# danping/CoSLAM

Hardware: AMD Instinct MI355X
Metric: frames/sec for track+local-BA loop, 8 cams 640x480 x 2000 feats (one frame = all 8 cameras) (higher is better)
Workload: dtype f32 (KLT, f16 pyramid storage) + f64 (pose, BA)

## Files before the change

coslam_amd/csrc/poseupdate.hip:

```cpp
#include <atomic>
#include <cstdlib>
#include <vector>

#include "cs_common.h"
#include "project_dev.h"
#include "triangulate_dev.h"
#include "history_view.h"
#include "register_rows_dev.h"
#include "small_ops.h"

#pragma clang fp contract(off)

namespace {

constexpr int PU_MAX_CAMS = 16;
constexpr int PU_MAX_HIST = 512;
constexpr int PU_MAX_STORE = 1 << 16;
constexpr int PU_LPS = 8;

struct PuArgs {
    int nCams, N, nMap, cam0, nCamsRun;
    int gateBlocks, dynBlocksPerCam;
    const int* pointFeat;
    const double* R;
// ... 2745 lines not shown
        return CS_ERR_INVALID;
    }
    if (!q.M || !q.cov || !q.pointFeat || !q.slot || !q.m || !q.var || !q.dist || !q.flags || q.M != d_mapPts || q.cov != d_mapCov ||
        q.pointFeat != d_pointFeat) {
        cs_set_error("cs_register_revisit_rounds_dev: the pass needs every table, and its map, covariances and feature table are the ones refined");
        return CS_ERR_INVALID;
    }
    if (nMap < 1 || cap < 1 || cap > RV_MAX_ROWS || nRounds < 1 || nRounds > 8 || kinds < 1 || kinds > 3 || mapBase < 0 || !(tolPix >= 0) ||
        !d_mapPts || !d_mapCov || !d_mergeCache || !d_mergeable || !d_rvLists || !d_rvCounts || !d_visitLoop || !d_nextLoop || !d_mapFlags ||
        !d_pointFeat || !d_slot2map || !d_attached || !d_regOut || !d_decideScratch || !d_curList || !d_curCount || !d_featRef ||
        (long long)nCams * N > RD_FEAT || (long long)nCams * nMap * nCams > 0x7fffffffLL) {
        cs_set_error("cs_register_revisit_rounds_dev: bad arguments (1..%d rows, 1..8 rounds, kinds 1..3, every table)", RV_MAX_ROWS);
        return CS_ERR_INVALID;
    }
    if (h->count < 1 || curFrame != h->lastFrame) {
        cs_set_error("cs_register_revisit_rounds_dev: the history's newest entry must be frame %d (it holds %d frame(s), the newest %d)", curFrame,
                     h->count, h->lastFrame);
        return CS_ERR_INVALID;
    }
    RrArgs A;
    memset((void*)&A, 0, sizeof(A));
    for (int c = 0; c < nCams; ++c) {
        const cs_register_cam& rc = regCams[c];
        if (!rc.K || !rc.R || !rc.t || !rc.xy || !rc.state || !rc.slot2map) {
            cs_set_error("cs_register_revisit_rounds_dev: null pointer in search camera %d", c);
            return CS_ERR_INVALID;
        }
        if (!cams[c].K || !cams[c].iK || !cams[c].trackSpan) {
            cs_set_error("cs_register_revisit_rounds_dev: null pointer in camera %d (K, iK, trackSpan are read)", c);
            return CS_ERR_INVALID;
        }
        if (!d_slot2map[c]) {
            cs_set_error("cs_register_revisit_rounds_dev: null slot2map of camera %d", c);
            return CS_ERR_INVALID;
        }
        A.rcam[c] = rc;
    }
    A.nRounds = nRounds, A.W = W, A.H = H, A.lists = d_rvLists, A.rvCounts = d_rvCounts;
    A.pass = q;
    A.pass.P = cap, A.pass.list = nullptr;
    MgCore& G = A.mg.a;
    G.cam0 = 0, G.nCams = nCams, G.N = N, G.P = nMap, G.H = h->H, G.head = h->head, G.nHist = hist_walk(h);
    G.sigma = pixelErrVar, G.M = d_mapPts, G.cov = d_mapCov, G.slot = q.slot, G.out = d_mergeable;
    G.histXY = h->xy, G.histR = h->R, G.histT = h->t;
    A.mg.W = hist_walk(h), A.mg.count = h->count, A.mg.curFrame = h->lastFrame, A.mg.epoch = h->tailEpoch, A.mg.fromMin = h->tailFromMin;
    A.mg.tolPix = tolPix, A.mg.cache = (MgCache*)d_mergeCache, A.mg.counts = nullptr, A.mg.flags = q.flags;
    RvArgs& V = A.rv;
    V.nCams = nCams, V.N = N, V.P = nMap, V.cap = cap, V.mapBase = mapBase, V.kinds = kinds, V.nextLoop = d_nextLoop, V.visitLoop = d_visitLoop;
    V.slot = q.slot, V.flags = q.flags, V.mergeable = d_mergeable, V.mapFlags = d_mapFlags, V.pointFeat = d_pointFeat;
    for (int c = 0; c < nCams; ++c) V.slot2map[c] = d_slot2map[c];
    V.attached = d_attached, V.regOut = d_regOut, V.curList = d_curList, V.curCount = d_curCount, V.curCap = curCap, V.counts = d_rvCnt;
    V.nextLoopW = d_nextLoop, V.overflow = d_rvCounts + nRounds;
    V.debug = cs_debug_get(CS_DBG_MERGE_PRINT) == 1;
    int* scr = (int*)d_decideScratch + (size_t)nCams * nMap + nMap;
    for (int k = 0; k < 3; ++k) V.owner[k] = scr, scr += (size_t)nCams * N;
    ArArgs& R = A.ar;
    R.nMap = nMap, R.featRef = (const int4*)d_featRef, R.mapPts = d_mapPts, R.mapCov = d_mapCov, R.sigma = pixelErrVar;
    R.refine = 1, R.select = d_regOut, R.selectW = d_regOut, R.clearSelect = 1;
    R.segPool = h->segPool, R.segCap = h->segCap, R.curFrame = h->lastFrame, R.stored = h->count < h->H ? h->count : h->H;
    R.nCams = nCams, R.N = N, R.H = h->H, R.head = h->head, R.nHist = hist_walk(h);
    R.histXY = h->xy, R.histR = h->R, R.histT = h->t, R.cen = h->cen;
    R.F.nCams = nCams, R.F.N = N, R.F.nMap = nMap, R.F.curFrame = curFrame, R.F.segCap = h->segCap;
    R.F.pointFeat = d_pointFeat, R.F.featRef = (int4*)d_featRef, R.F.refStatic = d_refStatic, R.F.segPool = h->segPool, R.F.segCount = h->segCount;
    R.F.counts = d_frefCounts;
    for (int c = 0; c < nCams; ++c) R.cam[c] = cams[c];
    CS_HIP(hipSetDevice(h->device));
    hipStream_t s = (hipStream_t)hip_stream;
    const int MC = nCams <= 8 ? 8 : RD_MAX_CAMS;
    const size_t lds = sizeof(double) * 12 * (size_t)A.mg.W + (cap > RR_THREADS ? sizeof(int) * (size_t)(MC + 1) * RV_MAX_ROWS : 0);
    size_t ldsMax = 0;
    if (const int rc = MC == 8 ? rr_dynamic_lds_limit<8>(h->device, &ldsMax) : rr_dynamic_lds_limit<RD_MAX_CAMS>(h->device, &ldsMax)) return rc;
    if (lds > ldsMax) {
        cs_set_error("cs_register_revisit_rounds_dev: %zu B of LDS (a history window of %d frames, lists of %d rows, %d cameras) where the "
                     "launch may carry %zu", lds, A.mg.W, cap, nCams, ldsMax);
        return CS_ERR_INVALID;
    }
    if (nMap > h->aliveCap) {
        if (h->alive) CS_HIP(hipFree(h->alive));
        h->alive = nullptr, h->aliveCap = 0;
        CS_HIP(hipMalloc((void**)&h->alive, (size_t)nMap));
        CS_HIP(hipMemsetAsync(h->alive, 1, (size_t)nMap, s));
        h->aliveCap = nMap;
    }
    R.F.alive = h->alive;
    hist_centres(h, s);
    if (MC == 8)
        hipLaunchKernelGGL(k_revisit_rounds<8>, dim3(1), dim3(RR_THREADS), lds, s, A);
    else
        hipLaunchKernelGGL(k_revisit_rounds<RD_MAX_CAMS>, dim3(1), dim3(RR_THREADS), lds, s, A);
    CS_HIP(hipGetLastError());
    return CS_OK;
}

extern "C" int cs_track_history_segments(const cs_track_history* h, cs_feat_seg** d_pool, int* cap, int** d_count) {
    if (!h) {
        cs_set_error("cs_track_history_segments: null handle");
        return CS_ERR_INVALID;
    }
    if (d_pool) *d_pool = (cs_feat_seg*)h->segPool;
    if (cap) *cap = h->segCap;
    if (d_count) *d_count = h->segCount;
    return CS_OK;
}

extern "C" int cs_track_history_segment_counts(const cs_track_history* h, int* counts) {
    if (!h || !counts) {
        cs_set_error("cs_track_history_segment_counts: bad arguments");
// ... 332 lines not shown
```

coslam_amd/csrc/register.hip:

```cpp
#include "cs_common.h"
#include "register_rows_dev.h"

#include <cfloat>

#pragma clang fp contract(off)

namespace {


struct RgArgs {
    int nCams, N, W, H, nPass, cam0;
    cs_register_pass pass[2];
    cs_register_cam cam[RG_MAX_CAMS];
};


constexpr int RG_WAVES = 8;
constexpr int RG_ROWS = RG_WAVES > 6 ? RG_WAVES : 6;
constexpr int RG_CHUNK = 512;

__global__ __launch_bounds__(64 * RG_WAVES) void k_register_search(RgArgs A) {
    extern __shared__ double lds[];
    CS_POSE_STREAM_PRIO();
    const int lane = threadIdx.x & 63, wave = threadIdx.x >> 6;
// ... 242 lines not shown
        const cs_register_cam& q = cams[c];
        if (!q.K || !q.R || !q.t || !q.xy || !q.state || !q.slot2map) {
            cs_set_error("cs_register_search_passes_dev: null pointer in camera %d", c);
            return CS_ERR_INVALID;
        }
        A.cam[c] = q;
    }
    CS_HIP(hipSetDevice(device));
    const int CH = N < RG_CHUNK ? N : RG_CHUNK;
    const size_t ldsBytes = (size_t)2 * CH * sizeof(double) + (size_t)RG_ROWS * 64 * sizeof(double) + (size_t)RG_WAVES * 64 * sizeof(int);
    hipLaunchKernelGGL(k_register_search, dim3((unsigned)((maxP + 63) / 64), (unsigned)nCamsRun, (unsigned)nPass), dim3(64 * RG_WAVES), ldsBytes,
                       (hipStream_t)hip_stream, A);
    CS_CHECK_LAUNCH();
    return CS_OK;
}

extern "C" int cs_register_search_dev(int device, void* hip_stream, int nCams, const cs_register_cam* cams, int N, int W, int H,
                                      int P, const double* d_M, const double* d_cov, const int* d_pointFeat, double sigmaSearch,
                                      double maxDist, double sigmaMerge, int* d_slot, double* d_m, double* d_var, double* d_dist,
                                      int* d_flags) {
    int rc = check_args("cs_register_search_dev", nCams, cams, N, W, H, P, sigmaSearch, maxDist, sigmaMerge);
    if (rc != CS_OK) return rc;
    if (P == 0) return CS_OK;
    if (!d_M || !d_cov || !d_pointFeat || !d_slot || !d_m || !d_var || !d_dist || !d_flags) {
        cs_set_error("cs_register_search_dev: null pointer");
        return CS_ERR_INVALID;
    }
    cs_register_pass q;
    memset(&q, 0, sizeof(q));
    q.P = P, q.sigmaSearch = sigmaSearch, q.maxDist = maxDist, q.sigmaMerge = sigmaMerge;
    q.M = d_M, q.cov = d_cov, q.pointFeat = d_pointFeat, q.slot = d_slot, q.m = d_m, q.var = d_var, q.dist = d_dist, q.flags = d_flags;
    return cs_register_search_passes_dev(device, hip_stream, nCams, cams, N, W, H, 1, &q);
}

namespace {

struct RdArgs {
    int nCams, N, P, mapBase, nSweeps, onlyCam, kinds;
    const int* slot;
    const int* flags;
    const unsigned char* mergeable;
    const unsigned char* mapFlags;
    int* pointFeat;
    int* slot2map[RD_MAX_CAMS];
    unsigned char* attached;
    unsigned char* regged;
    int* code;
    int* base;
    int* owner[3];
    int* counts;
    int* unconverged;
    int* timeouts;
    int* callFlag;
    int* changed;
    int* bar;
    int* rvLists;
    int* rvCounts;
    int rvCap, nRounds;
    int* visitLoop;
    int* nextLoop;
};
constexpr int RD_MAX_SWEEPS = 64;

__global__ __launch_bounds__(256) void k_decide_prepare(RdArgs A) {
    const int k = blockIdx.x * 256 + threadIdx.x, C = A.nCams, nFeat = C * A.N;
    for (int f = k; f < nFeat; f += gridDim.x * 256) A.owner[0][f] = RD_INF, A.owner[1][f] = RD_INF, A.owner[2][f] = RD_INF;
    if (k < 4 && A.counts) A.counts[k] = k == 2 ? A.nSweeps : (k == 3 ? 1 : 0);
    if (k == 0) *A.callFlag = 0, *A.bar = 0;
    if (k < RD_MAX_SWEEPS) A.changed[k] = 0;
    if (A.rvLists) {
        for (int f = k; f < A.nRounds * A.rvCap; f += gridDim.x * 256) A.rvLists[f] = -1;
        if (k < A.nRounds) A.rvCounts[k] = 0;
    }
    if (k >= A.P * C) return;
    const int p = k / C, i = k - p * C;
    A.attached[k] = 0;
    if (i == 0) A.regged[p] = 0;
    int code = -1;
    const unsigned char fl = A.mapFlags[p] & (CS_MAP_DYNAMIC | CS_MAP_FALSE | CS_MAP_UNCERTAIN);
    const int kind = (fl == 0 && (A.kinds & 1)) ? 0 : ((fl == CS_MAP_DYNAMIC && (A.kinds & 2)) ? 1 : -1);
    if (A.pointFeat[k] < 0 && kind >= 0) {
        const int s = A.slot[k];
        if (s >= 0 && s < A.N && ((A.flags[k] >> 1) & 1) == kind) {
            code = i * A.N + s;
            if (A.slot2map[i][s] >= 0) code |= RD_INIT_MAPPED;
            if (A.mergeable[k] == 1) code |= RD_CAN_MERGE;
        }
    }
    A.code[(size_t)i * A.P + p] = code;
    if (i == 0) {
        int ofirst = -1;
        for (int q = C - 1; q >= 0; --q)
            if (A.pointFeat[(size_t)p * C + q] >= 0) ofirst = q;
        if (A.onlyCam >= 0) ofirst = A.pointFeat[(size_t)p * C + A.onlyCam] >= 0 ? 0 : -1;
        A.base[p] = (ofirst >= 0 && kind >= 0) ? (ofirst * A.P + p) * C : -1;
    }
}
__global__ __launch_bounds__(256) void k_decide_sweep(RdArgs A, const int* __restrict__ prev, int* __restrict__ next, int* __restrict__ clear,
                                                      const int* __restrict__ prev2, int mode) {
    const int p = blockIdx.x * 256 + threadIdx.x, C = A.nCams, nFeat = C * A.N;
    if (clear)
        for (int f = p; f < nFeat; f += gridDim.x * 256) clear[f] = RD_INF;
    if (mode == 1 && prev2) {
        int ch = 0;
        for (int f = p; f < nFeat; f += gridDim.x * 256) ch |= prev[f] != prev2[f];
        if (ch) {
            if (A.counts) A.counts[3] = 0;
            if (atomicExch(A.callFlag, 1) == 0) atomicAdd(A.unconverged, 1);
        }
    }
    if (p >= A.P) return;
    const int base = A.base[p];
    if (base < 0) return;
    int code[RD_MAX_CAMS], own[RD_MAX_CAMS];
#pragma unroll
    for (int i = 0; i < RD_MAX_CAMS; ++i) code[i] = i < C ? A.code[(size_t)i * A.P + p] : -1;
#pragma unroll
    for (int i = 0; i < RD_MAX_CAMS; ++i) own[i] = code[i] >= 0 ? prev[code[i] & RD_FEAT] : RD_INF;
    bool go = true, reg = false;
    int nAtt = 0;
#pragma unroll
    for (int i = 0; i < RD_MAX_CAMS; ++i) {
        if (go && code[i] >= 0) {
            const int ord = base + i, f = code[i] & RD_FEAT;
            if ((code[i] & RD_INIT_MAPPED) || own[i] < ord) {
                go = false;
            } else if (code[i] & RD_CAN_MERGE) {
                if (mode == 0) {
                    atomicMin(&next[f], ord);
                } else if (own[i] == ord) {
                    const int s = f - i * A.N;
                    A.slot2map[i][s] = A.mapBase + p;
                    A.pointFeat[(size_t)p * C + i] = s;
                    A.attached[(size_t)p * C + i] = 1;
                    reg = true, ++nAtt;
                }
            }
        }
    }
    if (mode == 1 && reg) {
        A.regged[p] = 1;
        if (A.counts) atomicAdd(A.counts, nAtt), atomicAdd(A.counts + 1, 1);
    }
}

__device__ __forceinline__ bool rd_grid_barrier(int* ctr, int target) {
    __syncthreads();
    __shared__ int ok;
    if (threadIdx.x == 0) {
        __threadfence();
        atomicAdd(ctr, 1);
        const long long t0 = wall_clock64();
        int good = 1;
        while (__hip_atomic_load(ctr, __ATOMIC_ACQUIRE, __HIP_MEMORY_SCOPE_AGENT) < target) {
            __builtin_amdgcn_s_sleep(2);
            if (wall_clock64() - t0 > 2000000LL) {
                good = 0;
                break;
            }
        }
        ok = good;
    }
    __syncthreads();
    return ok != 0;
}

__global__ __launch_bounds__(256) void k_decide_settle(RdArgs A) {
    const int p = blockIdx.x * 256 + threadIdx.x, C = A.nCams, nFeat = C * A.N, nB = gridDim.x, stride = nB * 256;
    const int base = p < A.P ? A.base[p] : -1;
    int code[RD_MAX_CAMS];
#pragma unroll
    for (int i = 0; i < RD_MAX_CAMS; ++i) code[i] = (base >= 0 && i < C) ? A.code[(size_t)i * A.P + p] : -1;
    int arrivals = 0, k = 0;
    bool settled = false, alive = true;
    const int* fin = A.owner[0];
    for (; k < RD_MAX_SWEEPS; ++k) {
        const int* prev = A.owner[k % 3];
        int* next = A.owner[(k + 1) % 3];
        int* clear = A.owner[(k + 2) % 3];
        for (int f = p; f < nFeat; f += stride) rd_st(clear + f, RD_INF);
        if (base >= 0) {
            bool go = true;
#pragma unroll
            for (int i = 0; i < RD_MAX_CAMS; ++i) {
                if (go && code[i] >= 0) {
                    const int ord = base + i, f = code[i] & RD_FEAT;
                    if ((code[i] & RD_INIT_MAPPED) || rd_ld(prev + f) < ord) {
                        go = false;
                    } else if (code[i] & RD_CAN_MERGE) {
                        atomicMin(&next[f], ord);
                    }
                }
            }
        }
        arrivals += nB;
        if (!rd_grid_barrier(A.bar, arrivals)) {
            alive = false;
            break;
        }
        int ch = 0;
        for (int f = p; f < nFeat; f += stride) ch |= rd_ld(next + f) != rd_ld(prev + f);
        if (__syncthreads_or(ch) && threadIdx.x == 0) atomicOr(A.changed + k, 1);
        arrivals += nB;
        if (!rd_grid_barrier(A.bar, arrivals)) {
            alive = false;
            break;
        }
        fin = next;
        if (rd_ld(A.changed + k) == 0) {
            settled = true;
            ++k;
            break;
        }
    }
    if (p == 0 && A.counts) A.counts[2] = k, A.counts[3] = settled ? 1 : 0;
    if (!settled && p == 0) atomicAdd(A.unconverged, 1);
    if (!alive && p == 0) atomicAdd(A.timeouts, 1);
    if (!alive || base < 0) return;
    bool go = true, reg = false;
    int nAtt = 0;
#pragma unroll
    for (int i = 0; i < RD_MAX_CAMS; ++i) {
        if (go && code[i] >= 0) {
            const int ord = base + i, f = code[i] & RD_FEAT, own = rd_ld(fin + f);
            if ((code[i] & RD_INIT_MAPPED) || own < ord) {
                go = false;
            } else if ((code[i] & RD_CAN_MERGE) && own == ord) {
                const int s2 = f - i * A.N;
                A.slot2map[i][s2] = A.mapBase + p;
                A.pointFeat[(size_t)p * C + i] = s2;
                A.attached[(size_t)p * C + i] = 1;
                reg = true, ++nAtt;
            }
        }
    }
    if (reg) {
        A.regged[p] = 1;
        if (A.counts) atomicAdd(A.counts, nAtt), atomicAdd(A.counts + 1, 1);
        if (A.rvLists && A.onlyCam < 0) {
            const int last = (base / C) / A.P;
            A.visitLoop[p] = last;
            int b = -1;
            for (int c = C - 1; c > last; --c)
                if (A.pointFeat[(size_t)p * C + c] >= 0) b = c;
            if (b >= 0) {
                const int q = atomicAdd(A.rvCounts, 1);
                if (q < A.rvCap) A.rvLists[q] = p, A.nextLoop[p] = b;
                else atomicAdd(A.rvCounts + A.nRounds, 1);
            }
        }
    }
}

struct RvListArgs {
    int nCams, P, cap, firstRound;
    const int* pointFeat;
    const unsigned char* attached;
    unsigned char* regIn;
    int keepIn;
    unsigned char* regOutClear;
    int* visitLoop;
    int* nextLoop;
    int* list;
    int* counts;
};
__global__ __launch_bounds__(1024) void k_revisit_list(RvListArgs A) {
    __shared__ int sCount;
    const int tid = threadIdx.x, C = A.nCams;
    if (tid == 0) sCount = 0;
    __syncthreads();
    for (int p = tid; p < A.P; p += 1024) {
        if (A.regOutClear) A.regOutClear[p] = 0;
        if (!A.regIn[p]) continue;
        if (!A.keepIn) A.regIn[p] = 0;
        int last;
        if (A.firstRound) {
            last = -1;
            for (int c = C - 1; c >= 0; --c)
                if (A.pointFeat[(size_t)p * C + c] >= 0 && !A.attached[(size_t)p * C + c]) last = c;
            A.visitLoop[p] = last;
        } else {
            last = A.visitLoop[p];
        }
        if (last < 0) continue;
        int b = -1;
        for (int c = C - 1; c > last; --c)
            if (A.pointFeat[(size_t)p * C + c] >= 0) b = c;
        if (b < 0) continue;
        const int k = atomicAdd(&sCount, 1);
        if (k < A.cap) A.list[k] = p, A.nextLoop[p] = b;
    }
    __syncthreads();
    const int n = sCount < A.cap ? sCount : A.cap;
    for (int k = n + tid; k < A.cap; k += 1024) A.list[k] = -1;
    if (tid == 0 && A.counts) {
        A.counts[0] = n;
        if (sCount > A.cap) atomicAdd(A.counts + 1, sCount - A.cap);
    }
}

template <int MC>
__global__ __launch_bounds__(1024) void k_revisit_decide(RvArgs A) {
    if (A.listCount && *A.listCount == 0) return;
// ... 3 lines not shown
}

extern "C" int cs_register_revisit_list_dev(int device, void* hip_stream, int nCams, int P, int cap, int firstRound, const int* d_pointFeat,
                                            const unsigned char* d_attached, unsigned char* d_regIn, int keepIn, unsigned char* d_regOutClear,
                                            int* d_visitLoop, int* d_nextLoop, int* d_list, int* d_counts) {
    if (nCams < 1 || nCams > RD_MAX_CAMS || P < 1 || cap < 1 || cap > RV_MAX_ROWS || !d_pointFeat || !d_attached || !d_regIn || d_regOutClear == d_regIn || !d_visitLoop || !d_nextLoop ||
        !d_list) {
        cs_set_error("cs_register_revisit_list_dev: bad arguments (1..%d cameras, 1..%d rows)", RD_MAX_CAMS, RV_MAX_ROWS);
        return CS_ERR_INVALID;
    }
    RvListArgs A;
    A.nCams = nCams, A.P = P, A.cap = cap, A.firstRound = firstRound ? 1 : 0, A.pointFeat = d_pointFeat, A.attached = d_attached;
    A.regIn = d_regIn, A.keepIn = keepIn ? 1 : 0, A.regOutClear = d_regOutClear, A.visitLoop = d_visitLoop, A.nextLoop = d_nextLoop, A.list = d_list, A.counts = d_counts;
    CS_HIP(hipSetDevice(device));
    hipLaunchKernelGGL(k_revisit_list, dim3(1), dim3(1024), 0, (hipStream_t)hip_stream, A);
    CS_CHECK_LAUNCH();
    return CS_OK;
}

extern "C" int cs_register_revisit_decide_dev(int device, void* hip_stream, int nCams, int N, int P, int cap, int mapBase, int kinds, const int* d_list,
                                              const int* d_nextLoop, int* d_visitLoop, const int* d_slot, const int* d_flags,
                                              const unsigned char* d_mergeable, const unsigned char* d_mapFlags, int* d_pointFeat,
                                              int* const* d_slot2map, unsigned char* d_attached, unsigned char* d_regOut, void* d_decideScratch,
                                              const int* d_curList, const int* d_curCount, int curCap, int* d_counts, const int* d_listCount) {
    return cs_register_revisit_decide_next_dev(device, hip_stream, nCams, N, P, cap, mapBase, kinds, d_list, (int*)d_nextLoop, d_visitLoop, d_slot, d_flags,
                                               d_mergeable, d_mapFlags, d_pointFeat, d_slot2map, d_attached, d_regOut, d_decideScratch, d_curList, d_curCount,
                                               curCap, d_counts, d_listCount, nullptr, nullptr, nullptr);
}

extern "C" int cs_register_revisit_decide_next_dev(int device, void* hip_stream, int nCams, int N, int P, int cap, int mapBase, int kinds, const int* d_list,
                                                   int* d_nextLoop, int* d_visitLoop, const int* d_slot, const int* d_flags,
                                                   const unsigned char* d_mergeable, const unsigned char* d_mapFlags, int* d_pointFeat,
                                                   int* const* d_slot2map, unsigned char* d_attached, unsigned char* d_regOut, void* d_decideScratch,
                                                   const int* d_curList, const int* d_curCount, int curCap, int* d_counts, const int* d_listCount,
                                                   int* d_nextList, int* d_nextCount, int* d_overflow) {
    if ((d_nextList != nullptr) != (d_nextCount != nullptr)) {
        cs_set_error("cs_register_revisit_decide_next_dev: the next round's list and its count go together");
        return CS_ERR_INVALID;
    }
    if (nCams < 1 || nCams > RD_MAX_CAMS || N < 1 || P < 1 || cap < 1 || cap > RV_MAX_ROWS || kinds < 1 || kinds > 3 || !d_list || !d_nextLoop || !d_visitLoop ||
        !d_slot || !d_flags || !d_mergeable || !d_mapFlags || !d_pointFeat || !d_slot2map || !d_attached || !d_regOut || !d_decideScratch ||
        !d_curList || !d_curCount || (long long)nCams * N > RD_FEAT || (long long)nCams * P * nCams > 0x7fffffffLL) {
        cs_set_error("cs_register_revisit_decide_dev: bad arguments");
        return CS_ERR_INVALID;
    }
    RvArgs A;
    memset(&A, 0, sizeof(A));
    A.nCams = nCams, A.N = N, A.P = P, A.cap = cap, A.mapBase = mapBase, A.kinds = kinds, A.list = d_list, A.nextLoop = d_nextLoop, A.visitLoop = d_visitLoop;
    A.slot = d_slot, A.flags = d_flags, A.mergeable = d_mergeable, A.mapFlags = d_mapFlags, A.pointFeat = d_pointFeat;
    for (int c = 0; c < nCams; ++c) A.slot2map[c] = d_slot2map[c];
    A.attached = d_attached, A.regOut = d_regOut, A.curList = d_curList, A.curCount = d_curCount, A.curCap = curCap, A.counts = d_counts, A.listCount = d_listCount;
    A.nextList = d_nextList, A.nextCount = d_nextCount, A.nextLoopW = d_nextLoop, A.overflow = d_overflow;
    A.debug = cs_debug_get(CS_DBG_MERGE_PRINT) == 1;
    int* scr = (int*)d_decideScratch + (size_t)nCams * P + P;
    for (int k = 0; k < 3; ++k) A.owner[k] = scr, scr += (size_t)nCams * N;
    CS_HIP(hipSetDevice(device));
    if (nCams <= 8)
        hipLaunchKernelGGL(k_revisit_decide<8>, dim3(1), dim3(cap <= 256 ? 256 : (cap + 63) / 64 * 64), 0, (hipStream_t)hip_stream, A);
    else
        hipLaunchKernelGGL(k_revisit_decide<RD_MAX_CAMS>, dim3(1), dim3(cap <= 256 ? 256 : (cap + 63) / 64 * 64), 0, (hipStream_t)hip_stream, A);
    CS_CHECK_LAUNCH();
    return CS_OK;
}
extern "C" size_t cs_register_decide_scratch_bytes(int nCams, int N, int P) {
    if (nCams < 1 || N < 1 || P < 0) return 0;
    return sizeof(int) * ((size_t)nCams * P + (size_t)P + 3 * (size_t)nCams * N + RD_MAX_SWEEPS + 4);
}

extern "C" int cs_register_decide_static_dev(int device, void* hip_stream, int nCams, int N, int P, int mapBase, const int* d_slot, const int* d_flags,
                                             const unsigned char* d_mergeable, const unsigned char* d_mapFlags, int* d_pointFeat,
                                             int* const* d_slot2map , unsigned char* d_attached,
                                             unsigned char* d_regged, void* d_scratch, int nSweeps, int* d_counts) {
    return cs_register_decide_static_cam_dev(device, hip_stream, nCams, N, P, mapBase, d_slot, d_flags, d_mergeable, d_mapFlags, d_pointFeat, d_slot2map,
                                             d_attached, d_regged, d_scratch, nSweeps, d_counts, -1);
}

extern "C" int cs_register_decide_static_cam_dev(int device, void* hip_stream, int nCams, int N, int P, int mapBase, const int* d_slot,
                                                 const int* d_flags, const unsigned char* d_mergeable, const unsigned char* d_mapFlags,
                                                 int* d_pointFeat, int* const* d_slot2map, unsigned char* d_attached, unsigned char* d_regged,
                                                 void* d_scratch, int nSweeps, int* d_counts, int onlyCam) {
    return cs_register_decide_kinds_dev(device, hip_stream, nCams, N, P, mapBase, d_slot, d_flags, d_mergeable, d_mapFlags, d_pointFeat, d_slot2map,
                                        d_attached, d_regged, d_scratch, nSweeps, d_counts, onlyCam, 1);
}

extern "C" int cs_register_decide_kinds_dev(int device, void* hip_stream, int nCams, int N, int P, int mapBase, const int* d_slot, const int* d_flags,
                                            const unsigned char* d_mergeable, const unsigned char* d_mapFlags, int* d_pointFeat,
                                            int* const* d_slot2map, unsigned char* d_attached, unsigned char* d_regged, void* d_scratch,
                                            int nSweeps, int* d_counts, int onlyCam, int kinds) {
    return cs_register_decide_kinds_rounds_dev(device, hip_stream, nCams, N, P, mapBase, d_slot, d_flags, d_mergeable, d_mapFlags, d_pointFeat, d_slot2map,
                                               d_attached, d_regged, d_scratch, nSweeps, d_counts, onlyCam, kinds, nullptr, 0, 0, nullptr, nullptr, nullptr);
}

extern "C" int cs_register_decide_kinds_rounds_dev(int device, void* hip_stream, int nCams, int N, int P, int mapBase, const int* d_slot, const int* d_flags,
                                                   const unsigned char* d_mergeable, const unsigned char* d_mapFlags, int* d_pointFeat,
                                                   int* const* d_slot2map, unsigned char* d_attached, unsigned char* d_regged, void* d_scratch,
                                                   int nSweeps, int* d_counts, int onlyCam, int kinds, int* d_rvLists, int rvCap, int nRounds,
                                                   int* d_rvCounts, int* d_visitLoop, int* d_nextLoop) {
    if (d_rvLists && (rvCap < 1 || rvCap > RV_MAX_ROWS || nRounds < 1 || nRounds > 8 || !d_rvCounts || !d_visitLoop || !d_nextLoop || nSweeps != 0 || onlyCam >= 0)) {
        cs_set_error("cs_register_decide_kinds_rounds_dev: the second visits' lists need 1..%d rows, 1..8 rounds, their counters, visitLoop / nextLoop, "
                     "the self-settling launch (nSweeps 0) and all cameras' loops", RV_MAX_ROWS);
        return CS_ERR_INVALID;
    }
    if (onlyCam >= nCams || kinds < 1 || kinds > 3) {
        cs_set_error("cs_register_decide_kinds_dev: camera %d of %d, kinds %d (1: static, 2: dynamic, 3: both)", onlyCam, nCams, kinds);
        return CS_ERR_INVALID;
    }
    if (nCams < 1 || nCams > RD_MAX_CAMS || N < 1 || P < 0 || (long long)nCams * N > RD_FEAT || (long long)nCams * P * nCams > 0x7fffffffLL ||
        mapBase < 0 || nSweeps < 0 || nSweeps > 256 || !d_slot || !d_flags || !d_mergeable || !d_mapFlags || !d_pointFeat || !d_slot2map ||
        !d_attached || !d_regged || !d_scratch) {
        cs_set_error("cs_register_decide_static_dev: bad arguments (1..%d cameras, 0..256 sweeps)", RD_MAX_CAMS);
        return CS_ERR_INVALID;
    }
    RdArgs A;
    memset(&A, 0, sizeof(A));
    A.nCams = nCams, A.N = N, A.P = P, A.mapBase = mapBase, A.nSweeps = nSweeps, A.onlyCam = onlyCam < 0 ? -1 : onlyCam, A.kinds = kinds;
    A.slot = d_slot, A.flags = d_flags, A.mergeable = d_mergeable, A.mapFlags = d_mapFlags, A.pointFeat = d_pointFeat;
    for (int c = 0; c < nCams; ++c) {
        if (!d_slot2map[c]) {
            cs_set_error("cs_register_decide_static_dev: null slot2map of camera %d", c);
            return CS_ERR_INVALID;
        }
        A.slot2map[c] = d_slot2map[c];
    }
    A.attached = d_attached, A.regged = d_regged, A.counts = d_counts;
    A.rvLists = d_rvLists, A.rvCap = rvCap, A.nRounds = nRounds, A.rvCounts = d_rvCounts, A.visitLoop = d_visitLoop, A.nextLoop = d_nextLoop;
    int* scr = (int*)d_scratch;
    A.code = scr, scr += (size_t)nCams * P;
    A.base = scr, scr += P;
    for (int k = 0; k < 3; ++k) A.owner[k] = scr, scr += (size_t)nCams * N;
    A.changed = scr, scr += RD_MAX_SWEEPS;
    A.bar = scr, A.callFlag = scr + 1, A.timeouts = scr + 2, A.unconverged = scr + 3;
    CS_HIP(hipSetDevice(device));
    if (P == 0) return CS_OK;
    hipStream_t s = (hipStream_t)hip_stream;
    const int gE = (P * nCams + 255) / 256, gP = (P + 255) / 256;
    hipLaunchKernelGGL(k_decide_prepare, dim3(gE), dim3(256), 0, s, A);
    if (nSweeps == 0) {
        hipLaunchKernelGGL(k_decide_settle, dim3(gP), dim3(256), 0, s, A);
        CS_CHECK_LAUNCH();
        return CS_OK;
    }
    for (int k = 0; k < nSweeps; ++k)
        hipLaunchKernelGGL(k_decide_sweep, dim3(gP), dim3(256), 0, s, A, (const int*)A.owner[k % 3], A.owner[(k + 1) % 3], A.owner[(k + 2) % 3],
                           (const int*)nullptr, 0);
    hipLaunchKernelGGL(k_decide_sweep, dim3(gP), dim3(256), 0, s, A, (const int*)A.owner[nSweeps % 3], (int*)nullptr, (int*)nullptr,
                       (const int*)A.owner[(nSweeps + 2) % 3], 1);
    CS_CHECK_LAUNCH();
    return CS_OK;
}

namespace {

__global__ __launch_bounds__(256) void k_candidates_pack(int P, int nCams, int cam0, int nOwn, const int* __restrict__ slot, const int* __restrict__ flags,
                                                         const unsigned char* __restrict__ merg, int* __restrict__ send) {
    const int q = blockIdx.x * 256 + threadIdx.x;
    if (q >= nOwn * P) return;
    const int i = q / P, p = q - i * P;
    const size_t k = (size_t)p * nCams + cam0 + i;
    send[q] = slot[k], send[nOwn * P + q] = flags[k], send[2 * nOwn * P + q] = merg[k];
}
__global__ __launch_bounds__(256) void k_candidates_unpack(int P, int nCams, int nOwn, int skipRank, const int* __restrict__ recv, int* __restrict__ slot,
                                                           int* __restrict__ flags, unsigned char* __restrict__ merg) {
    const int q = blockIdx.x * 256 + threadIdx.x;
    if (q >= nCams * P) return;
    const int g = q / P, p = q - g * P, r = g / nOwn, i = g - r * nOwn;
    if (r == skipRank) return;
    const int* rec = recv + (size_t)r * 3 * nOwn * P;
    const size_t k = (size_t)p * nCams + g;
    slot[k] = rec[i * P + p], flags[k] = rec[nOwn * P + i * P + p], merg[k] = (unsigned char)rec[2 * nOwn * P + i * P + p];
}

}

namespace {
__global__ __launch_bounds__(256) void k_candidates_pack_list(int cap, int nCams, int cam0, int nOwn, const int* __restrict__ list,
                                                              const int* __restrict__ slot, const int* __restrict__ flags,
                                                              const unsigned char* __restrict__ merg, int* __restrict__ send) {
    const int q = blockIdx.x * 256 + threadIdx.x;
    if (q >= nOwn * cap) return;
    const int i = q / cap, j = q - i * cap, p = list[j];
    const size_t k = (size_t)(p < 0 ? 0 : p) * nCams + cam0 + i;
    send[q] = p < 0 ? -1 : slot[k], send[nOwn * cap + q] = p < 0 ? 0 : flags[k], send[2 * nOwn * cap + q] = p < 0 ? 255 : merg[k];
}
__global__ __launch_bounds__(256) void k_candidates_unpack_list(int cap, int nCams, int nOwn, int skipRank, const int* __restrict__ list,
                                                                const int* __restrict__ recv, int* __restrict__ slot, int* __restrict__ flags,
                                                                unsigned char* __restrict__ merg) {
    const int q = blockIdx.x * 256 + threadIdx.x;
    if (q >= nCams * cap) return;
    const int g = q / cap, j = q - g * cap, r = g / nOwn, i = g - r * nOwn, p = list[j];
    if (r == skipRank || p < 0) return;
    const int* rec = recv + (size_t)r * 3 * nOwn * cap;
// ... 152 lines not shown
```

coslam_amd/csrc/register_rows_dev.h:

```cpp
#pragma once

#include "cs_common.h"

#include <cfloat>

#pragma clang fp contract(off)

namespace {

constexpr int RG_MAX_CAMS = 16;

struct Proj {
    double u, v, w;
    double KR[9];
};

__device__ __forceinline__ void projection_cov(const Proj& q, const double* __restrict__ cov, double sigma, double var[4]) {
    const double ww = q.w * q.w;
    double J[6], JC[6];
#pragma unroll
    for (int j = 0; j < 3; ++j) {
        J[j] = (q.KR[j] * q.w - q.u * q.KR[6 + j]) / ww;
        J[3 + j] = (q.KR[3 + j] * q.w - q.v * q.KR[6 + j]) / ww;
    }
// ... 56 lines not shown
    return true;
}
__device__ __forceinline__ void rg_pair_finish(const cs_register_pass& Q, const cs_register_cam& C, int p, int N, const Proj& q, double m0,
                                               double m1, double dMin, int iMin, int& outSlot, int& outFlags, double& outDist) {
    if (iMin == 0x7fffffff) {
        outSlot = -4;
        return;
    }
    outSlot = iMin;
    outDist = dMin;
    if (C.slot2map[iMin] < 0) outFlags |= 1;
    if (C.isDynamic ? C.isDynamic[iMin] != 0 : (C.isStatic && C.isStatic[iMin] == 0)) outFlags |= 2;
    double v2[4], iv[4];
    projection_cov(q, Q.cov + 9 * (size_t)p, Q.sigmaMerge, v2);
    mat22_inv(v2, iv);
    if (!(maha_dist2(m0, m1, C.xy[iMin], C.xy[N + iMin], iv) > 1.0)) outFlags |= 4;
}
__device__ __forceinline__ void rg_pair_store(const cs_register_pass& Q, size_t o, int outSlot, int outFlags, double outDist, double m0, double m1,
                                              const double var[4]) {
    Q.slot[o] = outSlot;
    Q.flags[o] = outFlags;
    Q.dist[o] = outDist;
    Q.m[2 * o] = m0;
    Q.m[2 * o + 1] = m1;
#pragma unroll
    for (int k = 0; k < 4; ++k) Q.var[4 * o + k] = var[k];
}
__device__ __forceinline__ void rg_pair_scan_wave(const cs_register_cam& C, int N, int lane, double m0, double m1, const double ivar[4],
                                                  double& dMin, int& iMin) {
    dMin = DBL_MAX, iMin = 0x7fffffff;
    const double* __restrict__ xs = C.xy;
    const double* __restrict__ ys = C.xy + N;
    const int* __restrict__ st = C.state;
    for (int i = lane; i < N; i += 64) {
        const int s = st[i];
        if (s == 0 || s == 1) {
            const double d = maha_dist2(m0, m1, xs[i], ys[i], ivar);
            if (d < dMin) dMin = d, iMin = i;
        }
    }
#pragma unroll
    for (int off = 32; off > 0; off >>= 1) {
        const double d2 = __shfl_xor(dMin, off, 64);
        const int i2 = __shfl_xor(iMin, off, 64);
        if (d2 < dMin || (d2 == dMin && i2 < iMin)) dMin = d2, iMin = i2;
    }
}

constexpr int RD_MAX_CAMS = 16;
constexpr int RD_INIT_MAPPED = 1 << 29, RD_CAN_MERGE = 1 << 28, RD_FEAT = (1 << 28) - 1;
constexpr int RD_INF = 0x7fffffff;
__device__ __forceinline__ int rd_ld(const int* p) { return __hip_atomic_load(p, __ATOMIC_RELAXED, __HIP_MEMORY_SCOPE_AGENT); }
__device__ __forceinline__ void rd_st(int* p, int v) { __hip_atomic_store(p, v, __ATOMIC_RELAXED, __HIP_MEMORY_SCOPE_AGENT); }

struct RvArgs {
    int nCams, N, P, cap, mapBase, kinds;
    const int* list;
    const int* nextLoop;
    int* visitLoop;
    const int* slot;
    const int* flags;
    const unsigned char* mergeable;
    const unsigned char* mapFlags;
    int* pointFeat;
    int* slot2map[RD_MAX_CAMS];
    unsigned char* attached;
    unsigned char* regOut;
    int* owner[3];
    const int* curList;
    const int* curCount;
    int curCap;
    int* counts;
    const int* listCount;
    int* nextList;
    int* nextCount;
    int* nextLoopW;
    int* overflow;
    int debug;
};
constexpr int RV_MAX_ROWS = 1024;
struct RvRound {
    const int* list;
    const int* listCount;
    int* nextList;
    int* nextCount;
};
__device__ __forceinline__ RvRound rv_round_of(const RvArgs& A) { return RvRound{A.list, A.listCount, A.nextList, A.nextCount}; }
__device__ __forceinline__ int* rv_owner(const RvArgs& A, int k) {
    const int r = k % 3;
    return r == 0 ? A.owner[0] : (r == 1 ? A.owner[1] : A.owner[2]);
}
template <int MC>
__device__ __forceinline__ void rv_row_build(const RvArgs& A, int p, int (&code)[MC], int& base, int& nConf) {
    const int C = A.nCams;
    int kind = -1;
    base = -1;
#pragma unroll
    for (int i = 0; i < MC; ++i) code[i] = -1;
    int pfv[MC], slv[MC], flv[MC], own[MC];
    unsigned char mgv[MC];
    {
        const bool pv = p >= 0 && p < A.P;
        const size_t pr = pv ? (size_t)p : 0;
        const unsigned char fl = A.mapFlags[pr] & (CS_MAP_DYNAMIC | CS_MAP_FALSE | CS_MAP_UNCERTAIN);
        const int nl = A.nextLoop[pr];
#pragma unroll
// ... 298 lines not shown
```

Baseline: 2019.

## Replace grid-barrier settle kernel with last-block compacted active-list resolve

Removes the separate k_decide_settle kernel, which spun on software grid barriers across all blocks for each sweep. The prepare kernel now compacts the rows that could merge into an active list. The last block to finish, found through an atomic ticket, runs the owner-claim fixpoint alone with __syncthreads, using an LDS hash table when the set is small. This cuts a kernel launch and the grid-wide spin barriers. In exchange, a single block serialises the resolve, which could be slow if many rows are active, and the timeout accounting is gone.

```diff
diff --git a/coslam_amd/csrc/poseupdate.hip b/coslam_amd/csrc/poseupdate.hip
--- a/coslam_amd/csrc/poseupdate.hip
+++ b/coslam_amd/csrc/poseupdate.hip
@@ -2821,7 +2821,7 @@
     V.attached = d_attached, V.regOut = d_regOut, V.curList = d_curList, V.curCount = d_curCount, V.curCap = curCap, V.counts = d_rvCnt;
     V.nextLoopW = d_nextLoop, V.overflow = d_rvCounts + nRounds;
     V.debug = cs_debug_get(CS_DBG_MERGE_PRINT) == 1;
-    int* scr = (int*)d_decideScratch + (size_t)nCams * nMap + nMap;
+    int* scr = rd_scratch_owners(d_decideScratch, nCams, nMap);
     for (int k = 0; k < 3; ++k) V.owner[k] = scr, scr += (size_t)nCams * N;
     ArArgs& R = A.ar;
     R.nMap = nMap, R.featRef = (const int4*)d_featRef, R.mapPts = d_mapPts, R.mapCov = d_mapCov, R.sigma = pixelErrVar;
diff --git a/coslam_amd/csrc/register.hip b/coslam_amd/csrc/register.hip
--- a/coslam_amd/csrc/register.hip
+++ b/coslam_amd/csrc/register.hip
@@ -318,8 +318,9 @@
     int* unconverged;
     int* timeouts;
     int* callFlag;
-    int* changed;
-    int* bar;
+    int* ticket;
+    int* nActive;
+    int* active;
     int* rvLists;
     int* rvCounts;
     int rvCap, nRounds;
@@ -328,39 +329,242 @@
 };
 constexpr int RD_MAX_SWEEPS = 64;
 
-__global__ __launch_bounds__(256) void k_decide_prepare(RdArgs A) {
-    const int k = blockIdx.x * 256 + threadIdx.x, C = A.nCams, nFeat = C * A.N;
-    for (int f = k; f < nFeat; f += gridDim.x * 256) A.owner[0][f] = RD_INF, A.owner[1][f] = RD_INF, A.owner[2][f] = RD_INF;
-    if (k < 4 && A.counts) A.counts[k] = k == 2 ? A.nSweeps : (k == 3 ? 1 : 0);
-    if (k == 0) *A.callFlag = 0, *A.bar = 0;
-    if (k < RD_MAX_SWEEPS) A.changed[k] = 0;
+constexpr int RD_THREADS = 256;
+constexpr int RD_LDS_BITS = 10, RD_LDS_CELLS = 1 << RD_LDS_BITS, RD_LDS_ENTRIES = RD_LDS_CELLS / 2;
+
+__device__ __forceinline__ int* rd_owner(const RdArgs& A, int k) {
+    const int r = k % 3;
+    return r == 0 ? A.owner[0] : (r == 1 ? A.owner[1] : A.owner[2]);
+}
+template <int MC>
+__device__ __forceinline__ void rd_row_load(const RdArgs& A, int p, int (&code)[MC], int& base) {
+    base = p >= 0 ? rd_ld(A.base + p) : -1;
+#pragma unroll
+    for (int i = 0; i < MC; ++i) code[i] = (p >= 0 && i < A.nCams) ? rd_ld(A.code + (size_t)i * A.P + p) : -1;
+    bool go = base >= 0;
+#pragma unroll
+    for (int i = 0; i < MC; ++i) {
+        if (go && code[i] >= 0 && (code[i] & RD_INIT_MAPPED)) go = false;
+        if (!go) code[i] = -1;
+    }
+}
+template <int MC>
+__device__ __forceinline__ void rd_row_attach(const RdArgs& A, int p, const int (&code)[MC], int base, const int* fin, const int* keys) {
+    if (base < 0) return;
+    const int C = A.nCams;
+    bool go = true, reg = false;
+    int nAtt = 0;
+#pragma unroll
+    for (int i = 0; i < MC; ++i) {
+        if (go && code[i] >= 0) {
+            const int ord = base + i, cell = code[i] & RD_FEAT, own = rd_ld(fin + cell);
+            if (own < ord) {
+                go = false;
+            } else if ((code[i] & RD_CAN_MERGE) && own == ord) {
+                const int s2 = (keys ? keys[cell] : cell) - i * A.N;
+                A.slot2map[i][s2] = A.mapBase + p;
+                A.pointFeat[(size_t)p * C + i] = s2;
+                A.attached[(size_t)p * C + i] = 1;
+                reg = true, ++nAtt;
+            }
+        }
+    }
+    if (reg) {
+        A.regged[p] = 1;
+        if (A.counts) atomicAdd(A.counts, nAtt), atomicAdd(A.counts + 1, 1);
+        if (A.rvLists && A.onlyCam < 0) {
+            const int last = (base / C) / A.P;
+            A.visitLoop[p] = last;
+            int b = -1;
+            for (int c = C - 1; c > last; --c)
+                if (A.pointFeat[(size_t)p * C + c] >= 0) b = c;
+            if (b >= 0) {
+                const int q = atomicAdd(A.rvCounts, 1);
+                if (q < A.rvCap) A.rvLists[q] = p, A.nextLoop[p] = b;
+                else atomicAdd(A.rvCounts + A.nRounds, 1);
+            }
+        }
+    }
+}
+template <int MC>
+__device__ __forceinline__ void rd_resolve(const RdArgs& A, int n, int* sKey, int* sOwn) {
+    __shared__ int sChanged;
+    const int tid = threadIdx.x;
+    int code[MC], base = -1, k = 0;
+    bool settled = false;
+    if (n <= RD_THREADS && n * A.nCams <= RD_LDS_ENTRIES) {
+        for (int c = tid; c < RD_LDS_CELLS; c += RD_THREADS)
+            sKey[c] = -1, sOwn[c] = RD_INF, sOwn[RD_LDS_CELLS + c] = RD_INF, sOwn[2 * RD_LDS_CELLS + c] = RD_INF;
+        const int p = tid < n ? rd_ld(A.active + tid) : -1;
+        rd_row_load<MC>(A, p, code, base);
+        __syncthreads();
+#pragma unroll
+        for (int i = 0; i < MC; ++i) {
+            if (code[i] < 0) continue;
+            const int f = code[i] & RD_FEAT;
+            unsigned h = ((unsigned)f * 2654435761u) >> (32 - RD_LDS_BITS);
+            for (;;) {
+                const int old = atomicCAS(&sKey[h], -1, f);
+                if (old == -1 || old == f) break;
+                h = (h + 1) & (RD_LDS_CELLS - 1);
+            }
+            code[i] = (code[i] & ~RD_FEAT) | (int)h;
+        }
+        __syncthreads();
+        const int* fin = sOwn;
+        for (; k < RD_MAX_SWEEPS;) {
+            const int* prev = sOwn + (k % 3) * RD_LDS_CELLS;
+            int* next = sOwn + ((k + 1) % 3) * RD_LDS_CELLS;
+            int* clear = sOwn + ((k + 2) % 3) * RD_LDS_CELLS;
+            if (tid == 0) sChanged = 0;
+            rv_row_clear<MC>(code, base, clear);
+            __syncthreads();
+            rv_row_claim<MC>(code, base, prev, next);
+            __syncthreads();
+            if (rv_row_changed<MC>(code, base, prev, next)) sChanged = 1;
+            __syncthreads();
+            fin = next, ++k;
+            const int chg = sChanged;
+            __syncthreads();
+            if (!chg) {
+                settled = true;
+                break;
+            }
+        }
+        if (p >= 0) rd_row_attach<MC>(A, p, code, base, fin, sKey);
+    } else {
+        for (int j = tid; j < n; j += RD_THREADS) {
+            rd_row_load<MC>(A, rd_ld(A.active + j), code, base);
+#pragma unroll
+            for (int i = 0; i < MC; ++i)
+                if (code[i] >= 0) rd_st(A.owner[0] + (code[i] & RD_FEAT), RD_INF), rd_st(A.owner[1] + (code[i] & RD_FEAT), RD_INF), rd_st(A.owner[2] + (code[i] & RD_FEAT), RD_INF);
+        }
+        __syncthreads();
+        const int* fin = A.owner[0];
+        for (; k < RD_MAX_SWEEPS;) {
+            const int* prev = rd_owner(A, k);
+            int* next = rd_owner(A, k + 1);
+            int* clear = rd_owner(A, k + 2);
+            if (tid == 0) sChanged = 0;
+            for (int j = tid; j < n; j += RD_THREADS) {
+                rd_row_load<MC>(A, rd_ld(A.active + j), code, base);
+                rv_row_clear<MC>(code, base, clear);
+            }
+            __syncthreads();
+            for (int j = tid; j < n; j += RD_THREADS) {
+                rd_row_load<MC>(A, rd_ld(A.active + j), code, base);
+                rv_row_claim<MC>(code, base, prev, next);
+            }
+            __syncthreads();
+            int ch = 0;
+            for (int j = tid; j < n; j += RD_THREADS) {
+                rd_row_load<MC>(A, rd_ld(A.active + j), code, base);
+                ch |= rv_row_changed<MC>(code, base, prev, next);
+            }
+            if (ch) sChanged = 1;
+            __syncthreads();
+            fin = next, ++k;
+            const int chg = sChanged;
+            __syncthreads();
+            if (!chg) {
+                settled = true;
+                break;
+            }
+        }
+        for (int j = tid; j < n; j += RD_THREADS) {
+            const int p = rd_ld(A.active + j);
+            rd_row_load<MC>(A, p, code, base);
+            rd_row_attach<MC>(A, p, code, base, fin, nullptr);
+        }
+    }
+    if (tid == 0) {
+        if (A.counts) A.counts[2] = k, A.counts[3] = settled ? 1 : 0;
+        if (!settled) atomicAdd(A.unconverged, 1);
+    }
+}
+
+template <int MC>
+__global__ __launch_bounds__(RD_THREADS) void k_decide_prepare(RdArgs A) {
+    __shared__ int sCode[RD_THREADS];
+    __shared__ int sKey[RD_LDS_CELLS], sOwn[3 * RD_LDS_CELLS];
+    __shared__ int sCount, sFirst, sLast;
+    const int tid = threadIdx.x, C = A.nCams, nFeat = C * A.N, ppb = RD_THREADS / C;
+    const int g = blockIdx.x * RD_THREADS + tid, stride = gridDim.x * RD_THREADS;
+    const bool settle = A.nSweeps == 0;
+    if (!settle)
+        for (int f = g; f < nFeat; f += stride) A.owner[0][f] = RD_INF, A.owner[1][f] = RD_INF, A.owner[2][f] = RD_INF;
+    if (g < 4 && A.counts) rd_st(A.counts + g, g == 2 ? (settle ? 2 : A.nSweeps) : (g == 3 ? 1 : 0));
+    if (g == 0) *A.callFlag = 0;
     if (A.rvLists) {
-        for (int f = k; f < A.nRounds * A.rvCap; f += gridDim.x * 256) A.rvLists[f] = -1;
-        if (k < A.nRounds) A.rvCounts[k] = 0;
-    }
-    if (k >= A.P * C) return;
-    const int p = k / C, i = k - p * C;
-    A.attached[k] = 0;
-    if (i == 0) A.regged[p] = 0;
-    int code = -1;
-    const unsigned char fl = A.mapFlags[p] & (CS_MAP_DYNAMIC | CS_MAP_FALSE | CS_MAP_UNCERTAIN);
-    const int kind = (fl == 0 && (A.kinds & 1)) ? 0 : ((fl == CS_MAP_DYNAMIC && (A.kinds & 2)) ? 1 : -1);
-    if (A.pointFeat[k] < 0 && kind >= 0) {
-        const int s = A.slot[k];
-        if (s >= 0 && s < A.N && ((A.flags[k] >> 1) & 1) == kind) {
-            code = i * A.N + s;
-            if (A.slot2map[i][s] >= 0) code |= RD_INIT_MAPPED;
-            if (A.mergeable[k] == 1) code |= RD_CAN_MERGE;
-        }
-    }
-    A.code[(size_t)i * A.P + p] = code;
-    if (i == 0) {
-        int ofirst = -1;
-        for (int q = C - 1; q >= 0; --q)
-            if (A.pointFeat[(size_t)p * C + q] >= 0) ofirst = q;
-        if (A.onlyCam >= 0) ofirst = A.pointFeat[(size_t)p * C + A.onlyCam] >= 0 ? 0 : -1;
-        A.base[p] = (ofirst >= 0 && kind >= 0) ? (ofirst * A.P + p) * C : -1;
-    }
+        for (int f = g; f < A.nRounds * A.rvCap; f += stride) rd_st(A.rvLists + f, -1);
+        if (g < A.nRounds) rd_st(A.rvCounts + g, 0);
+    }
+    const int pl = tid / C, i = tid - pl * C, p = blockIdx.x * ppb + pl;
+    const bool live = pl < ppb && p < A.P;
+    int code = -1, base = -1;
+    if (live) {
+        const size_t k = (size_t)p * C + i;
+        rd_st8(A.attached + k, 0);
+        if (i == 0) rd_st8(A.regged + p, 0);
+        const unsigned char fl = A.mapFlags[p] & (CS_MAP_DYNAMIC | CS_MAP_FALSE | CS_MAP_UNCERTAIN);
+        const int kind = (fl == 0 && (A.kinds & 1)) ? 0 : ((fl == CS_MAP_DYNAMIC && (A.kinds & 2)) ? 1 : -1);
+        if (A.pointFeat[k] < 0 && kind >= 0) {
+            const int s = A.slot[k];
+            if (s >= 0 && s < A.N && ((A.flags[k] >> 1) & 1) == kind) {
+                code = i * A.N + s;
+                if (A.slot2map[i][s] >= 0) code |= RD_INIT_MAPPED;
+                if (A.mergeable[k] == 1) code |= RD_CAN_MERGE;
+            }
+        }
+        rd_st(A.code + (size_t)i * A.P + p, code);
+        if (i == 0) {
+            int ofirst = -1;
+            for (int q = C - 1; q >= 0; --q)
+                if (A.pointFeat[(size_t)p * C + q] >= 0) ofirst = q;
+            if (A.onlyCam >= 0) ofirst = A.pointFeat[(size_t)p * C + A.onlyCam] >= 0 ? 0 : -1;
+            base = (ofirst >= 0 && kind >= 0) ? (ofirst * A.P + p) * C : -1;
+            rd_st(A.base + p, base);
+        }
+    }
+    if (!settle) return;
+    sCode[tid] = code;
+    if (tid == 0) sCount = 0;
+    __syncthreads();
+    bool act = false;
+    if (base >= 0) {
+        for (int q = 0; q < C; ++q) {
+            const int c = sCode[tid + q];
+            if (c < 0) continue;
+            if (c & RD_INIT_MAPPED) break;
+            if (c & RD_CAN_MERGE) {
+                act = true;
+                break;
+            }
+        }
+    }
+    if (__syncthreads_or(act)) {
+        const int at = act ? atomicAdd(&sCount, 1) : 0;
+        __syncthreads();
+        if (tid == 0) sFirst = atomicAdd(A.nActive, sCount);
+        __syncthreads();
+        if (act && sFirst >= 0 && sFirst + at < A.P) rd_st(A.active + sFirst + at, p);
+    }
+    asm volatile("s_waitcnt vmcnt(0)" ::: "memory");
+    __syncthreads();
+    if (tid == 0) sLast = __hip_atomic_fetch_add(A.ticket, 1, __ATOMIC_RELAXED, __HIP_MEMORY_SCOPE_AGENT) == (int)gridDim.x - 1;
+    __syncthreads();
+    if (!sLast) return;
+    const int n = min(rd_ld(A.nActive), A.P);
+    if (n > 0) {
+        if (tid == 0) {
+            __builtin_amdgcn_fence(__ATOMIC_ACQUIRE, "agent");
+            asm volatile("s_waitcnt vmcnt(0)" ::: "memory");
+        }
+        __syncthreads();
+        rd_resolve<MC>(A, n, sKey, sOwn);
+    }
+    __syncthreads();
+    if (tid == 0) rd_st(A.ticket, 0), rd_st(A.nActive, 0);
 }
 __global__ __launch_bounds__(256) void k_decide_sweep(RdArgs A, const int* __restrict__ prev, int* __restrict__ next, int* __restrict__ clear,
                                                       const int* __restrict__ prev2, int mode) {
@@ -407,114 +611,6 @@
     if (mode == 1 && reg) {
         A.regged[p] = 1;
         if (A.counts) atomicAdd(A.counts, nAtt), atomicAdd(A.counts + 1, 1);
-    }
-}
-
-__device__ __forceinline__ bool rd_grid_barrier(int* ctr, int target) {
-    __syncthreads();
-    __shared__ int ok;
-    if (threadIdx.x == 0) {
-        __threadfence();
-        atomicAdd(ctr, 1);
-        const long long t0 = wall_clock64();
-        int good = 1;
-        while (__hip_atomic_load(ctr, __ATOMIC_ACQUIRE, __HIP_MEMORY_SCOPE_AGENT) < target) {
-            __builtin_amdgcn_s_sleep(2);
-            if (wall_clock64() - t0 > 2000000LL) {
-                good = 0;
-                break;
-            }
-        }
-        ok = good;
-    }
-    __syncthreads();
-    return ok != 0;
-}
-
-__global__ __launch_bounds__(256) void k_decide_settle(RdArgs A) {
-    const int p = blockIdx.x * 256 + threadIdx.x, C = A.nCams, nFeat = C * A.N, nB = gridDim.x, stride = nB * 256;
-    const int base = p < A.P ? A.base[p] : -1;
-    int code[RD_MAX_CAMS];
-#pragma unroll
-    for (int i = 0; i < RD_MAX_CAMS; ++i) code[i] = (base >= 0 && i < C) ? A.code[(size_t)i * A.P + p] : -1;
-    int arrivals = 0, k = 0;
-    bool settled = false, alive = true;
-    const int* fin = A.owner[0];
-    for (; k < RD_MAX_SWEEPS; ++k) {
-        const int* prev = A.owner[k % 3];
-        int* next = A.owner[(k + 1) % 3];
-        int* clear = A.owner[(k + 2) % 3];
-        for (int f = p; f < nFeat; f += stride) rd_st(clear + f, RD_INF);
-        if (base >= 0) {
-            bool go = true;
-#pragma unroll
-            for (int i = 0; i < RD_MAX_CAMS; ++i) {
-                if (go && code[i] >= 0) {
-                    const int ord = base + i, f = code[i] & RD_FEAT;
-                    if ((code[i] & RD_INIT_MAPPED) || rd_ld(prev + f) < ord) {
-                        go = false;
-                    } else if (code[i] & RD_CAN_MERGE) {
-                        atomicMin(&next[f], ord);
-                    }
-                }
-            }
-        }
-        arrivals += nB;
-        if (!rd_grid_barrier(A.bar, arrivals)) {
-            alive = false;
-            break;
-        }
-        int ch = 0;
-        for (int f = p; f < nFeat; f += stride) ch |= rd_ld(next + f) != rd_ld(prev + f);
-        if (__syncthreads_or(ch) && threadIdx.x == 0) atomicOr(A.changed + k, 1);
-        arrivals += nB;
-        if (!rd_grid_barrier(A.bar, arrivals)) {
-            alive = false;
-            break;
-        }
-        fin = next;
-        if (rd_ld(A.changed + k) == 0) {
-            settled = true;
-            ++k;
-            break;
-        }
-    }
-    if (p == 0 && A.counts) A.counts[2] = k, A.counts[3] = settled ? 1 : 0;
-    if (!settled && p == 0) atomicAdd(A.unconverged, 1);
-    if (!alive && p == 0) atomicAdd(A.timeouts, 1);
-    if (!alive || base < 0) return;
-    bool go = true, reg = false;
-    int nAtt = 0;
-#pragma unroll
-    for (int i = 0; i < RD_MAX_CAMS; ++i) {
-        if (go && code[i] >= 0) {
-            const int ord = base + i, f = code[i] & RD_FEAT, own = rd_ld(fin + f);
-            if ((code[i] & RD_INIT_MAPPED) || own < ord) {
-                go = false;
-            } else if ((code[i] & RD_CAN_MERGE) && own == ord) {
-                const int s2 = f - i * A.N;
-                A.slot2map[i][s2] = A.mapBase + p;
-                A.pointFeat[(size_t)p * C + i] = s2;
-                A.attached[(size_t)p * C + i] = 1;
-                reg = true, ++nAtt;
-            }
-        }
-    }
-    if (reg) {
-        A.regged[p] = 1;
-        if (A.counts) atomicAdd(A.counts, nAtt), atomicAdd(A.counts + 1, 1);
-        if (A.rvLists && A.onlyCam < 0) {
-            const int last = (base / C) / A.P;
-            A.visitLoop[p] = last;
-            int b = -1;
-            for (int c = C - 1; c > last; --c)
-                if (A.pointFeat[(size_t)p * C + c] >= 0) b = c;
-            if (b >= 0) {
-                const int q = atomicAdd(A.rvCounts, 1);
-                if (q < A.rvCap) A.rvLists[q] = p, A.nextLoop[p] = b;
-                else atomicAdd(A.rvCounts + A.nRounds, 1);
-            }
-        }
     }
 }
 
@@ -624,7 +720,7 @@
     A.attached = d_attached, A.regOut = d_regOut, A.curList = d_curList, A.curCount = d_curCount, A.curCap = curCap, A.counts = d_counts, A.listCount = d_listCount;
     A.nextList = d_nextList, A.nextCount = d_nextCount, A.nextLoopW = d_nextLoop, A.overflow = d_overflow;
     A.debug = cs_debug_get(CS_DBG_MERGE_PRINT) == 1;
-    int* scr = (int*)d_decideScratch + (size_t)nCams * P + P;
+    int* scr = rd_scratch_owners(d_decideScratch, nCams, P);
     for (int k = 0; k < 3; ++k) A.owner[k] = scr, scr += (size_t)nCams * N;
     CS_HIP(hipSetDevice(device));
     if (nCams <= 8)
@@ -636,7 +732,8 @@
 }
 extern "C" size_t cs_register_decide_scratch_bytes(int nCams, int N, int P) {
     if (nCams < 1 || N < 1 || P < 0) return 0;
-    return sizeof(int) * ((size_t)nCams * P + (size_t)P + 3 * (size_t)nCams * N + RD_MAX_SWEEPS + 4);
+    const size_t nList = (size_t)P > (size_t)RD_MAX_SWEEPS ? (size_t)P : (size_t)RD_MAX_SWEEPS;
+    return sizeof(int) * (RD_SCRATCH_HEAD + (size_t)nCams * P + (size_t)P + 3 * (size_t)nCams * N + nList + 4);
 }
 
 extern "C" int cs_register_decide_static_dev(int device, void* hip_stream, int nCams, int N, int P, int mapBase, const int* d_slot, const int* d_flags,
@@ -697,18 +794,21 @@
     A.attached = d_attached, A.regged = d_regged, A.counts = d_counts;
     A.rvLists = d_rvLists, A.rvCap = rvCap, A.nRounds = nRounds, A.rvCounts = d_rvCounts, A.visitLoop = d_visitLoop, A.nextLoop = d_nextLoop;
     int* scr = (int*)d_scratch;
+    A.ticket = scr, A.nActive = scr + 1, scr += RD_SCRATCH_HEAD;
     A.code = scr, scr += (size_t)nCams * P;
     A.base = scr, scr += P;
     for (int k = 0; k < 3; ++k) A.owner[k] = scr, scr += (size_t)nCams * N;
-    A.changed = scr, scr += RD_MAX_SWEEPS;
-    A.bar = scr, A.callFlag = scr + 1, A.timeouts = scr + 2, A.unconverged = scr + 3;
+    A.active = scr, scr += P > RD_MAX_SWEEPS ? P : RD_MAX_SWEEPS;
+    A.callFlag = scr + 1, A.timeouts = scr + 2, A.unconverged = scr + 3;
     CS_HIP(hipSetDevice(device));
     if (P == 0) return CS_OK;
     hipStream_t s = (hipStream_t)hip_stream;
-    const int gE = (P * nCams + 255) / 256, gP = (P + 255) / 256;
-    hipLaunchKernelGGL(k_decide_prepare, dim3(gE), dim3(256), 0, s, A);
+    const int ppb = RD_THREADS / nCams, gE = (P + ppb - 1) / ppb, gP = (P + 255) / 256;
+    if (nCams <= 8)
+        hipLaunchKernelGGL(k_decide_prepare<8>, dim3(gE), dim3(RD_THREADS), 0, s, A);
+    else
+        hipLaunchKernelGGL(k_decide_prepare<RD_MAX_CAMS>, dim3(gE), dim3(RD_THREADS), 0, s, A);
     if (nSweeps == 0) {
-        hipLaunchKernelGGL(k_decide_settle, dim3(gP), dim3(256), 0, s, A);
         CS_CHECK_LAUNCH();
         return CS_OK;
     }
diff --git a/coslam_amd/csrc/register_rows_dev.h b/coslam_amd/csrc/register_rows_dev.h
--- a/coslam_amd/csrc/register_rows_dev.h
+++ b/coslam_amd/csrc/register_rows_dev.h
@@ -132,6 +132,9 @@
 constexpr int RD_INF = 0x7fffffff;
 __device__ __forceinline__ int rd_ld(const int* p) { return __hip_atomic_load(p, __ATOMIC_RELAXED, __HIP_MEMORY_SCOPE_AGENT); }
 __device__ __forceinline__ void rd_st(int* p, int v) { __hip_atomic_store(p, v, __ATOMIC_RELAXED, __HIP_MEMORY_SCOPE_AGENT); }
+__device__ __forceinline__ void rd_st8(unsigned char* p, unsigned char v) { __hip_atomic_store(p, v, __ATOMIC_RELAXED, __HIP_MEMORY_SCOPE_AGENT); }
+constexpr int RD_SCRATCH_HEAD = 4;
+inline int* rd_scratch_owners(void* scratch, int nCams, int P) { return (int*)scratch + RD_SCRATCH_HEAD + (size_t)nCams * P + P; }
 
 struct RvArgs {
     int nCams, N, P, cap, mapBase, kinds;
```

Result: faster. 2062, median of 6 (+2.2%).
